# google/neural-light-transport

Hardware: AMD Instinct MI355X
Metric: rendered Mtexels/s at 1024^2 UV (full Model.call forward: U-Net + UV->camera warp); at N > 1: N collective-free replicas of this forward (weak scaling).  The data-parallel TRAIN step with the RCCL gradient all-reduce (BASELINE config 4) is `train_step`: value = Mtexels/s over all ranks, speedup_vs_o (higher is better)
Workload: dtype f32 via 3xbf16 split, 9 exact products, fp32 accumulate (the LDS-tiled encoder convs: fp32 operands as three bf16 terms on v_mfma_f32_16x16x32_bf16, every term product exact in fp32); f32 storage everywhere, every other launch native f32; 1 GPU; BASELINE config 3: dragon_specular relight+view-synth, depth0 16/depth 256, 4 frames/GPU, 1024^2 UV, k=4 obs maps, 512^2 camera warp; frames_per_gpu=4, uv=1024, k=4, cam=512, conv_algo=auto, plan=fused ends, launch=eager, two HIP streams, distinct_batches_rotated=3, launch_tape_replays=0, parallelism=dp1 (frames sharded, no forward collective), world=1, dist_world_size=1, device=cuda:0

## Files before the change

include/nlt_hip.h:

```cpp
#ifndef NLT_HIP_H_
#define NLT_HIP_H_

#ifdef __cplusplus
extern "C" {
#endif

typedef enum {
  NLT_OK = 0,
  NLT_ERR_BAD_ARG = -1,
  NLT_ERR_UNSUPPORTED = -2,
  NLT_ERR_LAUNCH = -3
} nlt_status;

typedef enum {
  NLT_CONV1X1 = 0,
  NLT_CONV_K2S2 = 1,
  NLT_CONV_K2S1 = 2,
  NLT_DECONV_K2S2 = 3,
  NLT_DECONV_K2S1 = 4,
  NLT_CONV_K3S1 = 5,
  NLT_CONV_K3S2 = 6,
  NLT_DECONV_K3S1 = 7,
  NLT_DECONV_K3S2 = 8
} nlt_conv_mode;

typedef enum {
  NLT_ALGO_AUTO = 0,
  NLT_ALGO_DIRECT = 1,
  NLT_ALGO_MFMA = 2
} nlt_conv_algo;

const char* nlt_version(void);
const char* nlt_status_string(int status);

long nlt_packed_weight_floats(int mode, int c0, int c1, int cout);

int nlt_pack_conv_weights(int mode, const float* w_keras, int c0, int c1, int cout,
                          float* w_packed, void* stream);

int nlt_conv_forward(int mode, int algo, int tile_hint,
                     const float* src0, int ld0, int c0,
                     const float* src1, int ld1, int c1,
                     int n, int h, int w,
                     const float* w_keras, const float* w_packed, const float* bias,
                     int cout, float* out, int ldo,
                     int act, float alpha,
                     const float* mask_src, int ldm, int accumulate,
                     void* stream);

int nlt_stem_forward(const float* base, const float* cvis, const float* lvis,
                     const float* nn_rgb, const float* nn_base, const float* obs_weights,
                     int n, int k, int h, int w, int c,
                     const float* wq, const float* bq, const float* wo, const float* bo,
                     float* fm0, float* obs0, void* stream);

int nlt_obs_mean_forward(const float* obs, const float* obs_weights, int n, int k, int hw, int c,
                         float* out, int ldo, void* stream);

int nlt_head_forward(const float* dec, int ldd, int cd, const float* skip, int lds, int cs,
                     const float* w_keras, const float* bias, const float* base,
                     int n, int h, int w, float* pred, void* stream);

int nlt_warp_forward(const float* pred, const float* base, const float* warp,
                     int n, int uvh, int uvw, int hc, int wc,
                     float* pred_cam, float* base_cam, float* fg_cam, int* idx_out, void* stream);

int nlt_warp_forward_store(const float* pred, const unsigned char* diffuse_store, const unsigned short* uv2cam_store,
                           const int* ids, int n, int uvh, int uvw, int hc, int wc,
                           float* pred_cam, float* base_cam, float* fg_cam, int* idx_out, void* stream);

int nlt_resample_forward(const float* data, const float* warp_px, int n, int h, int w, int c, int hc, int wc,
// ... 198 lines not shown
int nlt_front4_forward(const float* base, const float* cvis, const float* lvis, const float* nn_rgb,
                       const float* nn_base, int n, int k, int h, int w, const float* packed,
                       const float* packed_l2, int add_base, float alpha, float* fm1, float* skip3,
                       float* qtmp2, float* otmp2, int waves_per_simd, void* stream);
int nlt_front4_forward_u8(const unsigned char* diffuse_store, const unsigned char* rgb_store,
                          const unsigned char* cvis_store, const unsigned char* lvis_store,
                          const int* ids, const int* nn_ids, int n, int k, int h, int w,
                          const float* packed, const float* packed_l2, int add_base, float alpha,
                          float* fm1, float* skip3, float* qtmp2, float* otmp2, int waves_per_simd, void* stream);

int nlt_front4_forward_train(const float* base, const float* cvis, const float* lvis, const float* nn_rgb,
                             const float* nn_base, int n, int k, int h, int w, const float* packed,
                             const float* packed_l2, int add_base, float alpha, float* fm1, float* skip3,
                             float* qtmp2, float* otmp2, float* obs1, float* qtmp1, float* otmp1, void* stream);

int nlt_dec_block_forward(const float* x, int cx, const float* skip, int cs, int n, int h, int w,
                          const float* w_s2, const float* b_s2, const float* w_s1, const float* b_s1,
                          int c, float alpha, float* out, void* stream);

int nlt_back_forward(const float* x, const float* fm1, const float* skip3, int n, int h2, int w2,
                     const float* w_s2, const float* b_s2, const float* w_s1, const float* b_s1,
                     const float* w_head, float alpha, float* pred, void* stream);

typedef enum { NLT_REPACK_MFMA = 0, NLT_REPACK_TILE = 1, NLT_REPACK_WINO = 2 } nlt_repack_kind;
typedef struct {
  const float* src;
  float* dst;
  long total;
  long first_block;
  int kind, mode;
  int c0, c1, cout;
  int tn;
  int lo, full;
} nlt_repack_desc;
int nlt_repack_weights(const nlt_repack_desc* descs_device, int n_desc, long total_blocks, void* stream);

typedef struct {
  void* fn;
  int n_float, reserved;
  long iargs[32];
  float fargs[4];
} nlt_tape_call;
int nlt_tape_play(const nlt_tape_call* calls, int n, int* failed_index);
int nlt_event_create(int no_system_fence, void** event);
int nlt_event_destroy(void* event);
int nlt_event_record(void* event, void* stream);
int nlt_stream_wait_event(void* stream, void* event);

long nlt_wgrad_narrow_workspace_floats(int mode, int c0, int c1, int n, int h, int w, int cout);
int nlt_conv_backward_weights_narrow(int mode,
                                     const float* src0, int ld0, int c0, const float* src1, int ld1, int c1,
                                     int n, int h, int w, const float* dpre, int ldp, int cout,
                                     float* dw_keras, float* dbias, float* workspace, long workspace_floats,
                                     void* stream);

int nlt_front_forward_train(const float* base, const float* cvis, const float* lvis, const float* nn_rgb,
                            const float* nn_base, int n, int k, int h, int w, const float* packed,
                            int add_base, float alpha, float* fm1, float* obs1, float* skip3,
                            float* qtmp1, float* otmp1, void* stream);
int nlt_back_forward_train(const float* x, const float* fm1, const float* skip3, int n, int h2, int w2,
                           const float* w_s2, const float* b_s2, const float* w_s1, const float* b_s1,
                           const float* w_head, float alpha, float* pred, float* u, float* v, void* stream);

long nlt_front_backward_workspace_floats(int n, int h, int w);
int nlt_front_backward(const float* base, const float* cvis, const float* lvis, const float* nn_rgb,
                       const float* nn_base, int n, int k, int h, int w, const float* dy1q, const float* dy1o,
// ... 109 lines not shown
```

neural-light-transport_amd/_capi.py:

```python
import ctypes
import threading
import os

import torch

_HERE = os.path.dirname(os.path.abspath(__file__))
LIB_PATH = os.environ.get('NLT_HIP_LIB') or os.path.join(_HERE, 'libnlt_hip.so')

CONV1X1, CONV_K2S2, CONV_K2S1, DECONV_K2S2, DECONV_K2S1 = range(5)
CONV_K3S1, CONV_K3S2, DECONV_K3S1, DECONV_K3S2 = range(5, 9)
ALGO_AUTO, ALGO_DIRECT, ALGO_MFMA = range(3)

_c_int, _c_long, _c_float, _vp = ctypes.c_int, ctypes.c_long, ctypes.c_float, ctypes.c_void_p
_c_double = ctypes.c_double
MAP_F64, MAP_F32, MAP_F16 = range(3)

SIGNATURES = {
    'nlt_version': (ctypes.c_char_p, []),
    'nlt_status_string': (ctypes.c_char_p, [_c_int]),
    'nlt_packed_weight_floats': (_c_long, [_c_int] * 4),
    'nlt_pack_conv_weights': (_c_int, [_c_int, _vp, _c_int, _c_int, _c_int, _vp, _vp]),
    'nlt_conv_forward': (_c_int, [_c_int, _c_int, _c_int, _vp, _c_int, _c_int, _vp, _c_int, _c_int,
                                  _c_int, _c_int, _c_int, _vp, _vp, _vp, _c_int, _vp, _c_int,
                                  _c_int, _c_float, _vp, _c_int, _c_int, _vp]),
    'nlt_stem_forward': (_c_int, [_vp] * 6 + [_c_int] * 5 + [_vp] * 4 + [_vp, _vp, _vp]),
    'nlt_obs_mean_forward': (_c_int, [_vp, _vp, _c_int, _c_int, _c_int, _c_int, _vp, _c_int, _vp]),
    'nlt_head_forward': (_c_int, [_vp, _c_int, _c_int, _vp, _c_int, _c_int, _vp, _vp, _vp,
                                  _c_int, _c_int, _c_int, _vp, _vp]),
    'nlt_warp_forward': (_c_int, [_vp, _vp, _vp] + [_c_int] * 5 + [_vp] * 5),
    'nlt_warp_forward_store': (_c_int, [_vp] * 4 + [_c_int] * 5 + [_vp] * 5),
    'nlt_resample_forward': (_c_int, [_vp, _vp] + [_c_int] * 6 + [_vp, _vp]),
    'nlt_resize_bilinear_forward': (_c_int, [_vp] + [_c_int] * 6 + [_vp, _vp]),
    'nlt_mul_forward': (_c_int, [_vp, _vp, _c_long, _vp, _vp]),
    'nlt_conv_backward_weights': (_c_int, [_c_int, _c_int, _vp, _c_int, _c_int, _vp, _c_int, _c_int,
                                           _c_int, _c_int, _c_int, _vp, _c_int, _c_int, _vp, _vp, _vp]),
    'nlt_wgrad_workspace_floats': (_c_long, [_c_int] * 7),
    'nlt_conv_backward_weights_tiled': (_c_int, [_c_int, _vp, _c_int, _c_int, _vp, _c_int, _c_int, _c_int, _c_int, _c_int,
                                                 _vp, _c_int, _c_int, _vp, _vp, _vp, _c_long, _vp]),
    'nlt_repack_weights': (_c_int, [_vp, _c_int, _c_long, _vp]),
    'nlt_tape_play': (_c_int, [_vp, _c_int, _vp]),
    'nlt_event_create': (_c_int, [_c_int, _vp]),
    'nlt_event_destroy': (_c_int, [_vp]),
    'nlt_event_record': (_c_int, [_vp, _vp]),
    'nlt_stream_wait_event': (_c_int, [_vp, _vp]),
    'nlt_wgrad_narrow_workspace_floats': (_c_long, [_c_int] * 7),
    'nlt_conv_backward_weights_narrow': (_c_int, [_c_int, _vp, _c_int, _c_int, _vp, _c_int, _c_int, _c_int, _c_int, _c_int,
                                                 _vp, _c_int, _c_int, _vp, _vp, _vp, _c_long, _vp]),
    'nlt_lrelu_backward': (_c_int, [_vp, _c_int, _vp, _c_int, _c_int, _c_long, _c_float, _vp, _c_int, _vp]),
    'nlt_obs_mean_backward': (_c_int, [_vp, _c_int, _vp, _vp, _vp, _c_int, _c_int, _c_int, _c_int, _c_float, _vp, _vp]),
    'nlt_resize_cv_linear': (_c_int, [_vp, _c_int, _c_int, _c_int, _c_int, _c_int, _c_int, _c_int, _vp, _vp]),
    'nlt_l2_train_loss': (_c_int, [_vp, _vp, _vp, _c_int, _c_long, _c_float, _vp, _vp, _vp, _vp]),
    'nlt_level_split_backward': (_c_int, [_vp, _vp, _c_int, _vp, _vp, _vp, _c_int, _c_int, _c_int, _c_int, _c_float, _c_float, _vp, _vp]),
    'nlt_stem_backward': (_c_int, [_vp] * 6 + [_c_int] * 5 + [_vp] * 6 + [_vp]),
    'nlt_head_backward': (_c_int, [_vp, _c_int, _c_int, _vp, _c_int, _c_int, _vp, _vp, _c_int, _c_int, _c_int,
# ... 408 lines not shown
    if n <= 0:
        raise NLTError("%s%r: unsupported%s" % (name, args, ' (%s)' % what if what else ''))
    return n


_ws_cache = {}
_splitk_ws = _ws_cache


def _workspace(key, device, need, zero=False):
    key = (str(device),) + key if isinstance(key, tuple) else (str(device), key)
    ws = _ws_cache.get(key)
    if ws is None or ws.numel() < need:
        ws = (torch.zeros if zero else torch.empty)(need, device=device, dtype=torch.float32)
        _ws_cache[key] = ws
        _alloc_epoch[0] += 1
    return ws


def _per_stream(family):
    return '%s.%d' % (family, _stream())


def _pack(size_name, size_args, pack_name, pack_args, dtype, device):
    out = torch.empty(_size(size_name, *size_args), device=device, dtype=dtype)
    _call(pack_name, *pack_args, out.data_ptr())
    return out


def packed_weight_floats(mode, c0, c1, cout):
    return lib().nlt_packed_weight_floats(mode, c0, c1, cout)


def pack_conv_weights(mode, w_keras, c0, c1, cout):
    return _pack('nlt_packed_weight_floats', (mode, c0, c1, cout),
                 'nlt_pack_conv_weights', (mode, _ptr(_dense(w_keras, 'w_keras')), c0, c1, cout), torch.float32, w_keras.device)


def conv_forward(mode, src0, c0, ld0, src1, c1, ld1, n, h, w, w_keras, w_packed, bias, cout, out, ldo,
                 act=True, alpha=0.3, algo=ALGO_AUTO, tile_hint=0, mask_src=None, ldm=0, accumulate=False):
    _call('nlt_conv_forward', mode, algo, tile_hint, _ptr(src0), ld0, c0, _ptr(src1), ld1, c1, n, h, w, _ptr(w_keras),
          _ptr(w_packed), _ptr(bias), cout, _ptr(out), ldo, 1 if act else 0, float(alpha), _ptr(mask_src), ldm,
          1 if accumulate else 0)


def stem_forward(base, cvis, lvis, nn_rgb, nn_base, obs_weights, n, k, h, w, c, wq, bq, wo, bo, fm0, obs0):
    for t, nm in ((base, 'base'), (cvis, 'cvis'), (lvis, 'lvis'), (nn_rgb, 'nn_rgb'), (nn_base, 'nn_base')):
        _dense(t, nm)
    _call('nlt_stem_forward', _ptr(base), _ptr(cvis), _ptr(lvis), _ptr(nn_rgb), _ptr(nn_base), _ptr(obs_weights), n, k, h, w, c,
          _ptr(wq), _ptr(bq), _ptr(wo), _ptr(bo), _ptr(fm0), _ptr(obs0))


def obs_mean_forward(obs, obs_weights, n, k, hw, c, out, ldo):
    _call('nlt_obs_mean_forward', _ptr(_dense(obs, 'obs')), _ptr(obs_weights), n, k, hw, c, _ptr(out), ldo)


def head_forward(dec, ldd, cd, skip, lds, cs, w_keras, bias, base, n, h, w, pred):
    _call('nlt_head_forward', _ptr(dec), ldd, cd, _ptr(skip), lds, cs, _ptr(w_keras), _ptr(bias), _ptr(base), n, h, w, _ptr(pred))


def warp_forward(pred, base, warp, n, uvh, uvw, hc, wc, pred_cam, base_cam, fg_cam, idx_out=None):
    _call('nlt_warp_forward', _ptr(pred), _ptr(base), _ptr(_dense(warp, 'warp')), n, uvh, uvw, hc, wc, _ptr(pred_cam),
          _ptr(base_cam), _ptr(fg_cam), _ptr(idx_out))


def warp_forward_store(pred, diffuse_store, uv2cam_store, ids, n, uvh, uvw, hc, wc, pred_cam, base_cam, fg_cam, idx_out=None):
    if tuple(diffuse_store.shape[1:]) != (uvh, uvw, 3) or tuple(uv2cam_store.shape[1:]) != (hc, wc, 2):
# ... 365 lines not shown
    if abs(ksplit) <= 1 and not always:
        return None
    need = _size('nlt_conv_splitk_workspace_floats', mode, n, h, w, cout, ksplit)
    return _workspace((_stream(), getattr(_tls, 'scope', 0)), device, need, zero=True)


def conv_forward_splitk(mode, ksplit, src0, c0, ld0, src1, c1, ld1, n, h, w, w_packed, bias, cout, out, ldo,
                        act=True, alpha=0.3, tile_hint=0, mask_src=None, ldm=0, accumulate=False):
    ws = _splitk_workspace(mode, n, h, w, cout, ksplit, src0.device, always=True)
    _call('nlt_conv_forward_splitk', mode, tile_hint, ksplit, _ptr(ws), _ptr(src0), ld0, c0, _ptr(src1), ld1, c1, n, h, w,
          _ptr(w_packed), _ptr(bias), cout, _ptr(out), ldo, 1 if act else 0, float(alpha), _ptr(mask_src), ldm,
          1 if accumulate else 0)


def conv_forward_map(mode, ksplit, src0, c0, ld0, src1, c1, ld1, n, h, w, w_packed, bias, cout, out, ldo, bias_map,
                     act=True, alpha=0.3, tile_hint=0, w_keras=None):
    ws = _splitk_workspace(mode, n, h, w, cout, ksplit, src0.device)
    _call('nlt_conv_forward_map', mode, tile_hint, ksplit, _ptr(ws), _ptr(src0), ld0, c0, _ptr(src1), ld1, c1, n, h, w,
          _ptr(w_packed), _ptr(bias), cout, _ptr(out), ldo, 1 if act else 0, float(alpha), _ptr(_dense(bias_map, 'bias_map')),
          bias_map.shape[0])


def conv_backward_data(adj_mode, dpre, cpre, ldp, n, h, w, w_packed, zero_bias, cout, out, ldo, mask_src=None, ldm=0,
                       mask_alpha=0.3, accumulate=False, tile_hint=0, ksplit=1, split=None, w_keras=None):
    ws = _splitk_workspace(adj_mode, n, h, w, cout, ksplit, dpre.device)
    sc, sy, sd, sa, sp = split if split is not None else (0, None, None, 0.0, False)
    _call('nlt_conv_backward_data', adj_mode, tile_hint, ksplit, _ptr(ws), _ptr(dpre), ldp, cpre, n, h, w, _ptr(w_packed),
          _ptr(zero_bias), cout, _ptr(out), ldo, _ptr(mask_src), ldm, float(mask_alpha), 1 if accumulate else 0, sc, _ptr(sy),
          _ptr(sd), float(sa), 1 if sp else 0)


REPACK_MFMA, REPACK_TILE, REPACK_WINO = 0, 1, 2
REPACK_FIELDS = [('src', 'u8'), ('dst', 'u8'), ('total', 'i8'), ('first_block', 'i8'), ('kind', 'i4'), ('mode', 'i4'),
                 ('c0', 'i4'), ('c1', 'i4'), ('cout', 'i4'), ('tn', 'i4'), ('lo', 'i4'), ('full', 'i4')]


def repack_table(entries, device):
    import numpy as np
    tab = np.zeros(len(entries), dtype=np.dtype(REPACK_FIELDS))
    blocks = 0
    for i, e in enumerate(entries):
        if e['dst'].numel() % 4 or e['dst'].data_ptr() % 16:
            raise NLTError("repack_table: a packed buffer must be 16-byte aligned and a multiple of 4 floats long")
        tab[i] = (e['src'].data_ptr(), e['dst'].data_ptr(), e['dst'].numel(), blocks, e['kind'], e['mode'], e['c0'], e['c1'],
                  e['cout'], e['tn'], e['lo'], e['full'])
        blocks += (e['dst'].numel() + 255) // 256
    return torch.from_numpy(tab.view(np.uint8)).to(device), len(entries), blocks


def repack_weights(table, n_desc, total_blocks):
    _call('nlt_repack_weights', _tptr(table, torch.uint8, 'repack table'), n_desc, total_blocks)


def conv_tile_supported(mode, cin, cout, tn):
    return lib().nlt_conv_tile_packed_floats(mode, cin, cout, tn) > 0


def pack_conv_tile_weights(mode, w_keras, cin, cout, tn):
    return _pack('nlt_conv_tile_packed_floats', (mode, cin, cout, tn),
                 'nlt_pack_conv_tile_weights', (mode, _ptr(_dense(w_keras, 'w_keras')), cin, cout, tn), torch.float32, w_keras.device)


def conv_tile_forward(mode, src, ld, cin, frames, kobs, h, w, packed, bias, cout, tn, out, ldo, mean_out, ldm,
                      act=True, alpha=0.3):
    _call('nlt_conv_tile_forward', mode, _ptr(src), ld, cin, frames, kobs, h, w, _ptr(packed), _ptr(bias), cout, tn, _ptr(out), ldo,
          _ptr(mean_out), ldm, 1 if act else 0, float(alpha))


def pack_conv_tile_weights_adjoint(adj_mode, w_keras, cpre, cout, tn, full, lo):
    return _pack('nlt_conv_tile_packed_floats', (adj_mode, cpre, cout, tn), 'nlt_pack_conv_tile_weights_adjoint',
                 (adj_mode, _ptr(_dense(w_keras, 'w_keras')), cpre, cout, tn, full, lo), torch.float32, w_keras.device)


def conv_tile_backward_data(adj_mode, dpre, cpre, ldp, n, h, w, packed, cout, tn, out, ldo, mask_src=None, ldm=0, mask_alpha=0.3,
                            accumulate=False, split=None, w_keras=None):
    sc, sy, sd, sa, sp = split if split is not None else (0, None, None, 0.0, False)
    _call('nlt_conv_tile_backward_data', adj_mode, _ptr(dpre), ldp, cpre, n, h, w, _ptr(packed), cout, tn, _ptr(out), ldo,
          _ptr(mask_src), ldm, float(mask_alpha), 1 if accumulate else 0, sc, _ptr(sy), _ptr(sd), float(sa), 1 if sp else 0)
# ... 344 lines not shown
```

neural-light-transport_amd/csrc/conv_mfma.hip:

```cpp
#include "nlt_common.h"
#include "pack_common.h"

namespace {

typedef __attribute__((address_space(1))) unsigned gu32;

__host__ __device__ inline int chunks16(int c) { return (c + 15) >> 4; }

template <int MODE>
__device__ __forceinline__ int keras_widx(int t, int c, int ncol, int cin, int cout) {
  if (MODE == NLT_CONV1X1 || MODE == NLT_CONV_K2S2 || MODE == NLT_CONV_K2S1) return (t * cin + c) * cout + ncol;
  if (MODE == NLT_DECONV_K2S1) return (t * cout + ncol) * cin + c;
  return ncol * cin + c;
}

template <int MODE>
__global__ void pack_weights_kernel(const float* __restrict__ wk, int c0, int c1, int cout, int N,
                                    int ntiles, long total, float* __restrict__ wp) {
  const long idx = (long)blockIdx.x * blockDim.x + threadIdx.x;
  if (idx >= total) return;
  wp[idx] = nlt_mfma_fragment<MODE>(wk, idx, c0, c1, cout, N, ntiles, cout, 0);
}

template <int MODE>
__host__ __device__ inline int live_taps(const ConvP& p) {
  return ((MODE == NLT_CONV_K2S1 || MODE == NLT_DECONV_K2S1) && p.gh == 1 && p.gw == 1) ? 1 : ConvTraits<MODE>::TAPS;
}

__device__ __forceinline__ void split_store(const ConvP& p, int otex, int oc, f32x4 v) {
  const size_t at = (size_t)otex * p.split_c + (oc - p.split_c);
  f32x4* d = reinterpret_cast<f32x4*>(p.split_d + at);
  if (p.split_partial) v += *d;
  const f32x4 mk = *reinterpret_cast<const f32x4*>(p.split_y + at);
#pragma unroll
  for (int j = 0; j < 4; ++j) v[j] *= (mk[j] > 0.f) ? 1.f : p.split_alpha;
  *d = v;
}

template <int MODE, int RT, int CT, int PF, int NW>
__global__ __launch_bounds__(NW ? 64 * NW : 256) void conv_mfma_kernel(ConvP p, int mtiles, int ngroups, int ntiles, int ksplit,
                                                        float* ws) {
  const int lane = threadIdx.x & 63, wv = threadIdx.x >> 6;
  int ng, mt, ks, kg = 0, tile = 0;
  constexpr bool SPLIT = NW > 0;
  if constexpr (SPLIT) {
    const int kgroups = (ksplit + NW - 1) / NW;
    tile = blockIdx.x / kgroups;
    kg = blockIdx.x - tile * kgroups;
    ng = tile % ngroups;
    mt = tile / ngroups;
    ks = kg * NW + wv;
  } else {
    int wave = blockIdx.x * 4 + wv;
    ng = wave % ngroups; wave /= ngroups;
// ... 386 lines not shown
}

}

bool nlt_conv_mfma_supported(int mode, const ConvP& p) {
  (void)mode;
  if ((p.c0 & 3) || (p.c1 & 3) || (p.cout & 3) || (p.ld0 & 3) || (p.ldo & 3)) return false;
  if (p.c1 && (p.ld1 & 3)) return false;
  if (p.mask_src && (p.ldm & 3)) return false;
  if (!nlt_aligned16(p.src0) || !nlt_aligned16(p.out) || !nlt_aligned16(p.bias) || !nlt_aligned16(p.wgt)) return false;
  if (p.c1 && !nlt_aligned16(p.src1)) return false;
  if (p.mask_src && !nlt_aligned16(p.mask_src)) return false;
  return true;
}

int nlt_conv_mfma_launch(int mode, const ConvP& p, int tile_hint, hipStream_t s, int ksplit, float* ws) {
  if (!nlt_conv_mfma_supported(mode, p)) return NLT_ERR_UNSUPPORTED;
  switch (mode) {
    case NLT_CONV1X1: return launch_mode<NLT_CONV1X1>(p, tile_hint, ksplit, ws, s);
    case NLT_CONV_K2S2: return launch_mode<NLT_CONV_K2S2>(p, tile_hint, ksplit, ws, s);
    case NLT_CONV_K2S1: return launch_mode<NLT_CONV_K2S1>(p, tile_hint, ksplit, ws, s);
    case NLT_DECONV_K2S2: return launch_mode<NLT_DECONV_K2S2>(p, tile_hint, ksplit, ws, s);
    case NLT_DECONV_K2S1: return launch_mode<NLT_DECONV_K2S1>(p, tile_hint, ksplit, ws, s);
  }
  return NLT_ERR_BAD_ARG;
}

extern "C" long nlt_packed_weight_floats(int mode, int c0, int c1, int cout) {
  if (mode < NLT_CONV1X1 || mode > NLT_DECONV_K2S1 || c0 <= 0 || c1 < 0 || cout <= 0) return -1;
  const int N = (mode == NLT_DECONV_K2S2) ? 4 * cout : cout;
  return (long)taps_of(mode) * (chunks16(c0) + chunks16(c1)) * ((N + 15) >> 4) * 256;
}

extern "C" int nlt_pack_conv_weights(int mode, const float* w_keras, int c0, int c1, int cout,
                                     float* w_packed, void* stream) {
  if (!w_keras || !w_packed) return NLT_ERR_BAD_ARG;
  const long total = nlt_packed_weight_floats(mode, c0, c1, cout);
  if (total <= 0) return NLT_ERR_BAD_ARG;
  const int N = (mode == NLT_DECONV_K2S2) ? 4 * cout : cout;
  const int ntiles = (N + 15) >> 4;
  hipStream_t s = static_cast<hipStream_t>(stream);
  const unsigned blocks = (unsigned)((total + 255) / 256);
#define NLT_PACK(MODE) hipLaunchKernelGGL(pack_weights_kernel<MODE>, dim3(blocks), dim3(256), 0, s, w_keras, c0, c1, cout, N, ntiles, total, w_packed)
  switch (mode) {
    case NLT_CONV1X1: NLT_PACK(NLT_CONV1X1); break;
    case NLT_CONV_K2S2: NLT_PACK(NLT_CONV_K2S2); break;
    case NLT_CONV_K2S1: NLT_PACK(NLT_CONV_K2S1); break;
    case NLT_DECONV_K2S2: NLT_PACK(NLT_DECONV_K2S2); break;
    case NLT_DECONV_K2S1: NLT_PACK(NLT_DECONV_K2S1); break;
  }
#undef NLT_PACK
  NLT_CHECK_LAUNCH();
  return NLT_OK;
}
```

neural-light-transport_amd/csrc/pack_common.h:

```cpp
#pragma once
#include "nlt_common.h"

__host__ __device__ inline int nlt_chunks16(int c) { return (c + 15) >> 4; }

template <int MODE>
__device__ __forceinline__ long nlt_keras_widx(int t, int c, int ncol, int cin, int cout, int full, int lo) {
  if (MODE == NLT_CONV1X1 || MODE == NLT_CONV_K2S2 || MODE == NLT_CONV_K2S1) return ((long)t * cin + c) * full + lo + ncol;
  if (MODE == NLT_DECONV_K2S1) return ((long)t * full + lo + ncol) * cin + c;
  const int ab = ncol / cout, o = ncol - ab * cout;
  return ((long)ab * full + lo + o) * cin + c;
}

template <int MODE>
__device__ __forceinline__ float nlt_mfma_fragment(const float* __restrict__ wk, long idx, int c0, int c1, int cout, int N,
                                                   int ntiles, int full, int lo) {
  const int s4 = idx & 3;
  const int lane = (idx >> 2) & 63;
  const long tile = idx >> 8;
  const int nt = tile % ntiles;
  const int kc = tile / ntiles;
  const int ch0 = nlt_chunks16(c0), ch1 = nlt_chunks16(c1);
  const int t = kc / (ch0 + ch1);
  const int r = kc % (ch0 + ch1);
  const int s = r >= ch0;
  const int cl = (s ? r - ch0 : r) * 16 + 4 * (lane >> 4) + s4;
  const int cs = s ? c1 : c0;
  const int ncol = nt * 16 + (lane & 15);
  if (cl < cs && ncol < N) return wk[nlt_keras_widx<MODE>(t, (s ? c0 : 0) + cl, ncol, c0 + c1, cout, full, lo)];
  return 0.f;
}

__device__ __forceinline__ float nlt_tile_fragment(const float* __restrict__ wk, long idx, int cin, int cout, int tnt,
                                                   int full, int lo, bool transposed) {
  const int s4 = idx & 3, lane = (idx >> 2) & 63;
  long r = idx >> 8;
  const int ct = r % tnt; r /= tnt;
  const int t = r & 3; r >>= 2;
  const int ncc = cin >> 4;
  const int cc = r % ncc;
  const int g = r / ncc;
  const int c = cc * 16 + 4 * (lane >> 4) + s4;
  const int o = (g * tnt + ct) * 16 + (lane & 15);
  return transposed ? wk[((long)t * full + lo + o) * cin + c] : wk[((long)t * cin + c) * full + lo + o];
}

__device__ __forceinline__ float nlt_tile_fragment_d2(const float* __restrict__ wk, long idx, int cin, int cout, int tnt, int full, int lo) {
  const int s4 = idx & 3, lane = (idx >> 2) & 63;
  long r = idx >> 8;
  const int ct = r % tnt; r /= tnt;
  const int ncc = cin >> 4;
  const int cc = r % ncc;
  const int g = r / ncc;
  const int c = cc * 16 + 4 * (lane >> 4) + s4;
  const int col = (g * tnt + ct) * 16 + (lane & 15);
  const int ab = col / cout, o = col - ab * cout;
  return wk[((long)ab * full + lo + o) * cin + c];
}

__device__ __forceinline__ float nlt_wino_fragment(const float* __restrict__ wk, long idx, int cin, int cout, int tnt,
                                                   int full, int lo, bool transposed) {
  const int e = idx & 3, i = (idx >> 2) & 15, q = (idx >> 6) & 1;
// ... 18 lines not shown
```

neural-light-transport_amd/csrc/repack.hip:

```cpp
#include "pack_common.h"

namespace {

template <int MODE>
__device__ __forceinline__ float frag(const nlt_repack_desc& e, long idx) {
  const int N = MODE == NLT_DECONV_K2S2 ? 4 * e.cout : e.cout;
  return nlt_mfma_fragment<MODE>(e.src, idx, e.c0, e.c1, e.cout, N, (N + 15) >> 4, e.full, e.lo);
}

template <int MODE>
__device__ __forceinline__ f32x4 frag4(const nlt_repack_desc& e, long idx) {
  return (f32x4){frag<MODE>(e, idx), frag<MODE>(e, idx + 1), frag<MODE>(e, idx + 2), frag<MODE>(e, idx + 3)};
}

__global__ __launch_bounds__(64) void repack_all_kernel(const nlt_repack_desc* __restrict__ d, int nd) {
  int lo = 0, hi = nd;
  while (hi - lo > 1) {
    const int mid = (lo + hi) >> 1;
    if (d[mid].first_block <= (long)blockIdx.x) lo = mid; else hi = mid;
  }
  const nlt_repack_desc e = d[lo];
  const long idx = ((long)blockIdx.x - e.first_block) * 256 + threadIdx.x * 4;
  if (idx >= e.total) return;
  f32x4 v;
  if (e.kind == NLT_REPACK_WINO) {
    const bool tr = e.mode == NLT_DECONV_K2S1;
#pragma unroll
    for (int j = 0; j < 4; ++j) v[j] = nlt_wino_fragment(e.src, idx + j, e.c0, e.cout, e.tn >> 4, e.full, e.lo, tr);
  } else if (e.kind == NLT_REPACK_TILE && e.mode == NLT_DECONV_K2S2) {
#pragma unroll
    for (int j = 0; j < 4; ++j) v[j] = nlt_tile_fragment_d2(e.src, idx + j, e.c0, e.cout, e.tn >> 4, e.full, e.lo);
  } else if (e.kind == NLT_REPACK_TILE) {
    const bool tr = e.mode == NLT_DECONV_K2S1 || e.mode == NLT_DECONV_K2S2;
#pragma unroll
    for (int j = 0; j < 4; ++j) v[j] = nlt_tile_fragment(e.src, idx + j, e.c0, e.cout, e.tn >> 4, e.full, e.lo, tr);
  }
  else if (e.mode == NLT_CONV1X1) v = frag4<NLT_CONV1X1>(e, idx);
  else if (e.mode == NLT_CONV_K2S2) v = frag4<NLT_CONV_K2S2>(e, idx);
  else if (e.mode == NLT_CONV_K2S1) v = frag4<NLT_CONV_K2S1>(e, idx);
  else if (e.mode == NLT_DECONV_K2S2) v = frag4<NLT_DECONV_K2S2>(e, idx);
// ... 14 lines not shown
```

neural-light-transport_amd/engine.py:

```python
import os

import torch

from . import _capi as C
from .engine_infer import OverrideMixin


class OpTimer:

    def __init__(self):
        self.pending, self.records = [], {}
        self.flops = {}
        self.moved = {}

    def launch(self, label, nbytes, fn, *args, **kw):
        e0, e1 = torch.cuda.Event(enable_timing=True), torch.cuda.Event(enable_timing=True)
        e0.record()
        fn(*args, **kw)
        e1.record()
        self.pending.append((label, nbytes, e0, e1))

    def collect(self):
        torch.cuda.synchronize()
        for label, nbytes, e0, e1 in self.pending:
# ... 3 lines not shown
        self.pending = []
        return self.records


def _act_kw(act):
    return {'act': act is not None, 'alpha': act.alpha if act is not None else 0.0}


def _gemm(mode, n, h, w, cin, cout):
    ncols = cout * (4 if mode == C.DECONV_K2S2 else 1)
    taps = 4 if mode in (C.CONV_K2S2, C.CONV_K2S1, C.DECONV_K2S1) else 1
    rows = n * h * w // (4 if mode == C.CONV_K2S2 else 1)
    return rows, ncols, 2 * rows * taps * cin * ncols


class RenderPlan(OverrideMixin):
    def __init__(self, net_query, net_obs, use_obs=True):
        self.timer = None
        self.q, self.o, self.use_obs = net_query, net_obs, use_obs
        self.tile_hints = {}
        self.algo_hints = {}
        self.autotune = os.environ.get('NLT_AUTOTUNE', '1') != '0'
        self.fuse_ends = os.environ.get('NLT_FUSED', '1') != '0'
        self._front_blob = None
        self.fuse_override = os.environ.get('NLT_FUSED_OVERRIDE', '1') != '0'
        self._ovr = None
        self.front_l2 = os.environ.get('NLT_FRONT_L2', '1') != '0'
        self.fuse_dec = os.environ.get('NLT_FUSED_DEC', '1') != '0'
        self.front_v4 = os.environ.get('NLT_FRONT4', '1') != '0'
        self.fuse_train = os.environ.get('NLT_FUSED_TRAIN', '1') != '0'
        self.front4_train = os.environ.get('NLT_FRONT4_TRAIN', '1') != '0'
        self.two_streams = os.environ.get('NLT_STREAMS', '2') != '1'
        self._side = None
        self._bside = None
        self.wgrad_tiled = os.environ.get('NLT_WGRAD', 'tiled') != 'atomic'
        self.wgrad_narrow = os.environ.get('NLT_WGRAD_NARROW', '1') != '0'
        self.bwd_streams = int(os.environ.get('NLT_BWD_STREAMS', '1'))
        self.use_tape = os.environ.get('NLT_TAPE', '1') != '0'
        self.fold_split = os.environ.get('NLT_FOLD_SPLIT', '1') != '0'
        self.tile_dgrad = os.environ.get('NLT_TILE_DGRAD', '1') != '0'
        self._tuning = False
        self.tune_backward = os.environ.get('NLT_TUNE_BWD', '1') != '0'
        self.precision = os.environ.get('NLT_PRECISION', 'fp32')
        self._pred_out = None
        self._pred_slot = 'back_infer'
        self.prune_packs = os.environ.get('NLT_PRUNE_PACKS', '1') != '0'
        self.grad_hook = None
        self.grad_mid_level = 0
        self.generation = 0
        self.tape_replays = 0
        self._trial_direct = False
        self._ran_direct = set()
        self._trial_lds = 0
        self._ran_lds = set()
        self.lds_hints = {}
        self.use_wino = os.environ.get('NLT_WINO', '1') != '0'
        self._trial_wino = 0
        self._ran_wino = set()
        self.wino_hints = {}
        self.use_c32 = os.environ.get('NLT_C32', '1') != '0'
        self._trial_c32 = 0
        self._ran_c32 = set()
        self.c32_hints = {}
        self.alias_obs = os.environ.get('NLT_ALIAS_OBS', '1') != '0'
        self._trial_splitk = 0
        self._ran_splitk = set()
        self.splitk_hints = {}
        is_c = net_query.is_contracting
        self.n_down = sum(is_c) - 1
        self.n_up = len(is_c) - sum(is_c) - 1
        assert self.n_down == self.n_up
        self._bufs = {}
# ... 46 lines not shown
            if moved is not None:
                t.moved[label] = moved
        if t is not None and (getattr(t, 'only', None) is None or label in t.only):
            t.launch(label, nbytes, fn, *args, **kw)
        else:
            fn(*args, **kw)

    def _tile_splitk(self, label, rows, ncols, star, trial):
        tile_hint = self.tile_hints.get(label, self.tile_hints.get('*', 0) if star else 0)
        if tile_hint and ((ncols + 15) // 16) % (tile_hint & 15):
            tile_hint = 0
        ks = self.splitk_hints.get(label, 1)
        if trial:
            rt, ct = (tile_hint >> 4, tile_hint & 15) if tile_hint else (1, 1)
            waves = -(-rows // (16 * rt)) * (-(-ncols // 16) // ct)
            npad = -(-ncols // 16) * 16
            ks = self._trial_splitk if (waves < 4096 and rows * npad * abs(self._trial_splitk) <= (1 << 24)) else 1
        return tile_hint, ks

    def _conv(self, label, layer, act, src0, c0, ld0, src1, c1, ld1, n, h, w, out, ldo, algo=C.ALGO_AUTO, bmap=None):
        layer.build(c0 + c1, src0.device)
        assert layer.cin == c0 + c1, (layer.cin, c0, c1)
        small = (c0 + c1) * layer.n_ch_out <= 1024
        if self.algo_hints.get(label) == C.ALGO_DIRECT or (self._trial_direct and small):
            algo = C.ALGO_DIRECT
            self._ran_direct.add(label)
        ok = c0 % 4 == 0 and c1 % 4 == 0 and layer.n_ch_out % 4 == 0 and algo != C.ALGO_DIRECT
        oh, ow = layer.out_hw(h, w)
        nbytes = 4 * (n * h * w * (c0 + c1) + n * oh * ow * layer.n_ch_out)
        rows, ncols, flops = _gemm(layer.mode, n, h, w, c0 + c1, layer.n_ch_out)
        if c1 == 0 and ok and algo == C.ALGO_AUTO and self._wino(label, layer, act, src0, c0, ld0, n, 1, h, w, out, ldo):
            return
        tile_hint, ks = self._tile_splitk(label, rows, ncols, True, self._trial_splitk and ok)
        srcs = (src0, c0, ld0, src1, c1, ld1, n, h, w)
        dst = (layer.bias.detach(), layer.n_ch_out, out, ldo)
        kw = dict(_act_kw(act), flops=flops)
        if bmap is not None:
            if not ok:
                raise C.NLTError("a bias-map conv needs channel counts that are multiples of 4 (%s)" % label)
            if abs(ks) > 1:
                self._ran_splitk.add(label)
            self._launch(label, nbytes, C.conv_forward_map, layer.mode, ks or 1, *srcs, layer.packed(c0, c1), *dst, bmap,
                         tile_hint=tile_hint, w_keras=layer.kernel.detach(), **kw)
        elif abs(ks) > 1 and ok:
            self._ran_splitk.add(label)
            self._launch(label, nbytes, C.conv_forward_splitk, layer.mode, ks, *srcs, layer.packed(c0, c1), *dst,
                         tile_hint=tile_hint, **kw)
        else:
            self._launch(label, nbytes, C.conv_forward, layer.mode, *srcs, layer.kernel.detach(),
                         layer.packed(c0, c1) if ok else None, *dst, algo=algo if ok else C.ALGO_DIRECT,
                         tile_hint=tile_hint if ok else 0, **kw)

    def _mean(self, label, obs, obs_weights, frames, kobs, hw, c, mean_out, ldm):
        self._launch(label.replace('.s1', '.mean'), 4 * frames * hw * c * (kobs + 1), C.obs_mean_forward,
                     obs, obs_weights, frames, kobs, hw, c, mean_out, ldm)

    def _enc_launch(self, fn, packed, extra, ran, unfold, label, layer, act, src, cin, ld, frames, kobs, h, w, out, ldo,
                    mean_out, ldm, **kw):
        oh, ow = layer.out_hw(h, w)
        nf, c = frames * kobs, layer.n_ch_out
        fold_mean = mean_out is not None and not unfold
        nbytes = 4 * (nf * h * w * cin + nf * oh * ow * c)
        if fold_mean:
            nbytes += 4 * frames * oh * ow * c * (kobs + 1)
        ran.add(label)
        self._launch(label, nbytes, fn, layer.mode, src, ld, cin, nf if unfold else frames, 1 if unfold else kobs, h, w, packed,
                     layer.bias.detach(), c, *extra, out, ldo, mean_out if fold_mean else None, ldm, **_act_kw(act), **kw,
                     flops=2 * nf * oh * ow * 4 * cin * c)
        if mean_out is not None and unfold:
            self._mean(label, out, None, frames, kobs, oh * ow, c, mean_out, ldm)

    def _wino(self, label, layer, act, src, cin, ld, frames, kobs, h, w, out, ldo, mean_out=None, ldm=0, obs_weights=None):
        hint = self._trial_wino or self.wino_hints.get(label, 0)
        tn, unfold = hint & 255, bool(hint >> 8)
        if not (tn and self.use_wino and obs_weights is None and layer.mode in (C.CONV_K2S1, C.DECONV_K2S1) and layer.cin == cin
                and cin % 8 == 0 and layer.n_ch_out % tn == 0 and ld % 4 == 0 and ldo % 4 == 0):
            return False
        if layer.mode == C.DECONV_K2S1 and (kobs > 1 or mean_out is not None):
            return False
        if kobs == 1 and mean_out is None:
            if self._trial_wino >> 8:
                return False
            unfold = False
        self._enc_launch(C.conv_wino_forward, layer.packed_wino(tn), (tn,), self._ran_wino, unfold, label, layer, act, src, cin, ld,
                         frames, kobs, h, w, out, ldo, mean_out, ldm)
        return True

    def _conv_bf(self, label, layer, act, src0, c0, ld0, src1, c1, ld1, n, h, w, out, ldo):
# ... 434 lines not shown
            h2_, w2_ = hh // 2, ww // 2

            def obs_path():
                if bf and l >= 3:
                    self._conv_bf('L%d.o.s2' % l, oa, oact_a, b['obs'][l - 1], cl[l - 1], cl[l - 1], None, 0, 0, n * k, hh, ww,
                                  b['otmp'][l], c)
                    self._conv_bf('L%d.o.s1' % l, ob, oact_b, b['otmp'][l], c, c, None, 0, 0, n * k, h2_, w2_, b['obs'][l], c)
                    self._launch('L%d.o.mean' % l, 4 * n * h2_ * w2_ * c * (k + 1), C.obs_mean_bf16, b['obs'][l], n, k, h2_ * w2_, c,
                                 b['fm'][l].view(-1)[c:], 2 * c, moved=2 * n * h2_ * w2_ * c * (k + 1))
                    return
                if alias_obs:
                    if not s2_done:
                        if l > 2:
                            self._conv_enc('L%d.o.s2' % l, oa, oact_a, b['fm'][l - 1].view(-1)[cl[l - 1]:], cl[l - 1], 2 * cl[l - 1],
                                           n, 1, hh, ww, b['otmp'][l], c, algo)
                        else:
                            self._conv_enc('L%d.o.s2' % l, oa, oact_a, b['obs'][1], cl[1], cl[1], n, 1, hh, ww, b['otmp'][l], c, algo)
                    self._conv_enc('L%d.o.s1' % l, ob, oact_b, b['otmp'][l], c, c, n, 1, h2_, w2_, b['fm'][l].view(-1)[c:], 2 * c, algo)
                    return
                if not s2_done:
                    self._conv_enc('L%d.o.s2' % l, oa, oact_a, b['obs'][l - 1], cl[l - 1], cl[l - 1], n, k, hh, ww, b['otmp'][l], c, algo)
                self._conv_enc('L%d.o.s1' % l, ob, oact_b, b['otmp'][l], c, c, n, k, h2_, w2_, b['obs'][l], c, algo,
                               mean_out=b['fm'][l].view(-1)[c:], ldm=2 * c)

            def query_path():
                if bf and l >= 3:
                    self._conv_bf('L%d.q.s2' % l, qa, qact_a, b['fm'][l - 1], cin, cin, None, 0, 0, n, hh, ww, b['qtmp'][l], c)
                    self._conv_bf('L%d.q.s1' % l, qb, qact_b, b['qtmp'][l], c, c, None, 0, 0, n, h2_, w2_, b['fm'][l], 2 * c)
                    return
                if not s2_done:
                    self._conv_enc('L%d.q.s2' % l, qa, qact_a, b['fm'][l - 1], cin, cin, n, 1, hh, ww, b['qtmp'][l], c, algo)
                self._conv_enc('L%d.q.s1' % l, qb, qact_b, b['qtmp'][l], c, c, n, 1, h2_, w2_, b['fm'][l], 2 * c, algo)

            obs_path()
            if concurrent:
                C.record_event(ev[l], main)
                with torch.cuda.stream(side):
                    if l > 2:
                        C.wait_event(side, ev[l - 1])
                    query_path()
            else:
                query_path()
            hh, ww = hh // 2, ww // 2
        if concurrent:
            C.record_event(ev[D + 1], side)
            C.wait_event(main, ev[D + 1])
        x, cx = b['fm'][D], 2 * cl[D]
        for j in range(U - 1):
            (da, dact_a), (db, dact_b) = q.layers[D + 1 + j].convs()
            skip, cs = b['fm'][D - j], 2 * cl[D - j]
            lab = 'L%d.q' % (D + 1 + j)
            nl = da.n_ch_out
            if bf and j <= D - 3:
                self._conv_bf(lab + '.s2', da, dact_a, x, cx, cx, skip, cs, cs, n, hh, ww, b['dtmp'][j], nl)
                hh, ww = hh * 2, ww * 2
                self._conv_bf(lab + '.s1', db, dact_b, b['dtmp'][j], nl, nl, None, 0, 0, n, hh, ww, b['dec'][j], db.n_ch_out)
                x, cx = b['dec'][j], db.n_ch_out
                continue
            if (self.fuse_dec and not train and nl in (8, 16) and db.n_ch_out == nl and cx % 4 == 0 and algo == C.ALGO_AUTO
                    and dact_a is not None and dact_b is not None and dact_a.alpha == dact_b.alpha and not self._trial_direct):
                da.build(cx + cs, dev); db.build(nl, dev)
                nbytes = 4 * n * hh * ww * ((cx + cs) + 4 * nl) + 4 * n * 4 * hh * ww * 2 * nl
                self._launch(lab, nbytes, C.dec_block_forward, x, cx, skip, cs, n, hh, ww, da.kernel.detach(), da.bias.detach(),
                             db.kernel.detach(), db.bias.detach(), nl, dact_a.alpha, b['dec'][j],
                             flops=2 * n * hh * ww * (cx + cs) * 4 * nl + 2 * n * 4 * hh * ww * 4 * nl * nl,
                             moved=4 * n * hh * ww * ((cx + cs) + 4 * nl))
                hh, ww = hh * 2, ww * 2
                x, cx = b['dec'][j], nl
                continue
            x, cx = self._dec_block_plain(b, j, lab, da, dact_a, db, dact_b, (x, cx, cx, skip, cs, cs), n, hh, ww, algo)
            hh, ww = hh * 2, ww * 2
        (da, _), (db, _) = q.layers[D + U].convs()
        head = q.layers[-1]
# ... 295 lines not shown
```

neural-light-transport_amd/networks/elements.py:

```python
import math

import torch

from .. import _capi as C

_seed_counter = [0]


def _glorot_uniform(shape, device, seed):
    kh, kw, a, b = shape
    limit = math.sqrt(6.0 / (kh * kw * a + kh * kw * b))
    g = torch.Generator().manual_seed(seed)
    return ((torch.rand(shape, generator=g) * 2 - 1) * limit).to(device)


class Layer:
    built = True
    trainable = ()

    def build(self, cin, device):
        return cin

    def variables(self):
        return []
# ... 60 lines not shown
    def _version(self):
        return (self.kernel.data_ptr(), self.kernel._version, self._epoch[0])

    def _cached_pack(self, key, make, desc):
        ent = self._packed.get(key)
        ver = self._version()
        reg = self._registry
        if reg is not None:
            reg.touch(self, key)
            if ent is not None and reg.is_inactive(self, key):
                paused = C.tape_pause()
                try:
                    reg.activate(self, key)
                    ent[1].copy_(make())
                finally:
                    C.tape_resume(paused)
                self._packed[key] = (ver, ent[1])
                return ent[1]
        if ent is not None and ent[0] == ver:
            return ent[1]
        if ent is not None and reg is not None and reg.owns(self, key):
            paused = C.tape_pause()
            try:
                reg.refresh()
            finally:
                C.tape_resume(paused)
            return self._packed[key][1]
        buf = make()
        self._packed[key] = (ver, buf)
        if reg is not None:
            reg.add(self, key, buf, desc)
        return buf

    def packed(self, c0, c1):
        return self._cached_pack((c0, c1), lambda: C.pack_conv_weights(self.mode, self.kernel.detach(), c0, c1, self.n_ch_out),
                                 dict(kind=C.REPACK_MFMA, mode=self.mode, c0=c0, c1=c1, cout=self.n_ch_out, tn=0, lo=0,
                                      full=self.n_ch_out))

    def packed_tile(self, tn):
        return self._cached_pack(('tile', tn),
                                 lambda: C.pack_conv_tile_weights(self.mode, self.kernel.detach(), self.cin, self.n_ch_out, tn),
                                 dict(kind=C.REPACK_TILE, mode=self.mode, c0=self.cin, c1=0, cout=self.n_ch_out, tn=tn, lo=0,
                                      full=self.n_ch_out))

    def packed_wino(self, tn):
        return self._cached_pack(('wino', tn),
                                 lambda: C.pack_conv_wino_weights(self.mode, self.kernel.detach(), self.cin, self.n_ch_out, tn),
                                 dict(kind=C.REPACK_WINO, mode=self.mode, c0=self.cin, c1=0, cout=self.n_ch_out, tn=tn, lo=0,
                                      full=self.n_ch_out))

    def packed_adjoint_wino(self, lo, hi, tn):
        adj = self.ADJOINT[self.mode]
        return self._cached_pack(('adjwino', lo, hi, tn),
                                 lambda: C.pack_conv_wino_weights(adj, self.kernel.detach(), self.n_ch_out, hi - lo, tn, self.cin, lo),
                                 dict(kind=C.REPACK_WINO, mode=adj, c0=self.n_ch_out, c1=0, cout=hi - lo, tn=tn, lo=lo, full=self.cin))

    def packed_bf16(self, c0, c1):
        cache = self.__dict__.setdefault('_packed_bf', {})
        ent, ver = cache.get((c0, c1)), self._version()
        if ent is None or ent[0] != ver:
            ent = cache[(c0, c1)] = (ver, C.conv_bf16_pack(self.mode, self.kernel.detach(), c0, c1, self.n_ch_out))
        return ent[1]

    def packed_tile3(self, tn):
        cache = self.__dict__.setdefault('_packed_t3', {})
        ent, ver = cache.get(tn), self._version()
        if ent is None or ent[0] != ver:
            ent = cache[tn] = (ver, C.pack_conv_tile3_weights(self.mode, self.kernel.detach(), self.cin, self.n_ch_out, tn))
        return ent[1]

# ... 348 lines not shown
```

Baseline: 3451 Mtexels/s.

## Fold duplicated concat sources into summed weights and move obs means to side stream

```diff
diff --git a/include/nlt_hip.h b/include/nlt_hip.h
--- a/include/nlt_hip.h
+++ b/include/nlt_hip.h
@@ -37,6 +37,9 @@
 
 int nlt_pack_conv_weights(int mode, const float* w_keras, int c0, int c1, int cout,
                           float* w_packed, void* stream);
+
+int nlt_pack_conv_weights_fold(int mode, const float* w_keras, int c0, int fold, int cout,
+                               float* w_packed, void* stream);
 
 int nlt_conv_forward(int mode, int algo, int tile_hint,
                      const float* src0, int ld0, int c0,
@@ -301,6 +304,8 @@
   int c0, c1, cout;
   int tn;
   int lo, full;
+  int fold;
+  int reserved;
 } nlt_repack_desc;
 int nlt_repack_weights(const nlt_repack_desc* descs_device, int n_desc, long total_blocks, void* stream);
 
diff --git a/neural-light-transport_amd/_capi.py b/neural-light-transport_amd/_capi.py
--- a/neural-light-transport_amd/_capi.py
+++ b/neural-light-transport_amd/_capi.py
@@ -20,6 +20,7 @@
     'nlt_status_string': (ctypes.c_char_p, [_c_int]),
     'nlt_packed_weight_floats': (_c_long, [_c_int] * 4),
     'nlt_pack_conv_weights': (_c_int, [_c_int, _vp, _c_int, _c_int, _c_int, _vp, _vp]),
+    'nlt_pack_conv_weights_fold': (_c_int, [_c_int, _vp, _c_int, _c_int, _c_int, _vp, _vp]),
     'nlt_conv_forward': (_c_int, [_c_int, _c_int, _c_int, _vp, _c_int, _c_int, _vp, _c_int, _c_int,
                                   _c_int, _c_int, _c_int, _vp, _vp, _vp, _c_int, _vp, _c_int,
                                   _c_int, _c_float, _vp, _c_int, _c_int, _vp]),
@@ -494,7 +495,12 @@
     return lib().nlt_packed_weight_floats(mode, c0, c1, cout)
 
 
-def pack_conv_weights(mode, w_keras, c0, c1, cout):
+def pack_conv_weights(mode, w_keras, c0, c1, cout, fold=0):
+    if fold:
+        if c1:
+            raise NLTError("pack_conv_weights: a folded pack has one source (c1 = %d)" % c1)
+        return _pack('nlt_packed_weight_floats', (mode, c0, 0, cout), 'nlt_pack_conv_weights_fold',
+                     (mode, _ptr(_dense(w_keras, 'w_keras')), c0, fold, cout), torch.float32, w_keras.device)
     return _pack('nlt_packed_weight_floats', (mode, c0, c1, cout),
                  'nlt_pack_conv_weights', (mode, _ptr(_dense(w_keras, 'w_keras')), c0, c1, cout), torch.float32, w_keras.device)
 
@@ -926,7 +932,8 @@
 
 REPACK_MFMA, REPACK_TILE, REPACK_WINO = 0, 1, 2
 REPACK_FIELDS = [('src', 'u8'), ('dst', 'u8'), ('total', 'i8'), ('first_block', 'i8'), ('kind', 'i4'), ('mode', 'i4'),
-                 ('c0', 'i4'), ('c1', 'i4'), ('cout', 'i4'), ('tn', 'i4'), ('lo', 'i4'), ('full', 'i4')]
+                 ('c0', 'i4'), ('c1', 'i4'), ('cout', 'i4'), ('tn', 'i4'), ('lo', 'i4'), ('full', 'i4'), ('fold', 'i4'),
+                 ('reserved', 'i4')]
 
 
 def repack_table(entries, device):
@@ -937,7 +944,7 @@
         if e['dst'].numel() % 4 or e['dst'].data_ptr() % 16:
             raise NLTError("repack_table: a packed buffer must be 16-byte aligned and a multiple of 4 floats long")
         tab[i] = (e['src'].data_ptr(), e['dst'].data_ptr(), e['dst'].numel(), blocks, e['kind'], e['mode'], e['c0'], e['c1'],
-                  e['cout'], e['tn'], e['lo'], e['full'])
+                  e['cout'], e['tn'], e['lo'], e['full'], e.get('fold', 0), 0)
         blocks += (e['dst'].numel() + 255) // 256
     return torch.from_numpy(tab.view(np.uint8)).to(device), len(entries), blocks
 
diff --git a/neural-light-transport_amd/csrc/conv_mfma.hip b/neural-light-transport_amd/csrc/conv_mfma.hip
--- a/neural-light-transport_amd/csrc/conv_mfma.hip
+++ b/neural-light-transport_amd/csrc/conv_mfma.hip
@@ -16,10 +16,10 @@
 
 template <int MODE>
 __global__ void pack_weights_kernel(const float* __restrict__ wk, int c0, int c1, int cout, int N,
-                                    int ntiles, long total, float* __restrict__ wp) {
+                                    int ntiles, long total, float* __restrict__ wp, int fold) {
   const long idx = (long)blockIdx.x * blockDim.x + threadIdx.x;
   if (idx >= total) return;
-  wp[idx] = nlt_mfma_fragment<MODE>(wk, idx, c0, c1, cout, N, ntiles, cout, 0);
+  wp[idx] = nlt_mfma_fragment<MODE>(wk, idx, c0, c1, cout, N, ntiles, cout, 0, fold);
 }
 
 template <int MODE>
@@ -472,16 +472,17 @@
   return (long)taps_of(mode) * (chunks16(c0) + chunks16(c1)) * ((N + 15) >> 4) * 256;
 }
 
-extern "C" int nlt_pack_conv_weights(int mode, const float* w_keras, int c0, int c1, int cout,
-                                     float* w_packed, void* stream) {
-  if (!w_keras || !w_packed) return NLT_ERR_BAD_ARG;
+namespace {
+
+int pack_conv_weights(int mode, const float* w_keras, int c0, int c1, int fold, int cout, float* w_packed, void* stream) {
+  if (!w_keras || !w_packed || fold < 0) return NLT_ERR_BAD_ARG;
   const long total = nlt_packed_weight_floats(mode, c0, c1, cout);
   if (total <= 0) return NLT_ERR_BAD_ARG;
   const int N = (mode == NLT_DECONV_K2S2) ? 4 * cout : cout;
   const int ntiles = (N + 15) >> 4;
   hipStream_t s = static_cast<hipStream_t>(stream);
   const unsigned blocks = (unsigned)((total + 255) / 256);
-#define NLT_PACK(MODE) hipLaunchKernelGGL(pack_weights_kernel<MODE>, dim3(blocks), dim3(256), 0, s, w_keras, c0, c1, cout, N, ntiles, total, w_packed)
+#define NLT_PACK(MODE) hipLaunchKernelGGL(pack_weights_kernel<MODE>, dim3(blocks), dim3(256), 0, s, w_keras, c0, c1, cout, N, ntiles, total, w_packed, fold)
   switch (mode) {
     case NLT_CONV1X1: NLT_PACK(NLT_CONV1X1); break;
     case NLT_CONV_K2S2: NLT_PACK(NLT_CONV_K2S2); break;
@@ -493,3 +494,16 @@
   NLT_CHECK_LAUNCH();
   return NLT_OK;
 }
+
+}
+
+extern "C" int nlt_pack_conv_weights(int mode, const float* w_keras, int c0, int c1, int cout,
+                                     float* w_packed, void* stream) {
+  return pack_conv_weights(mode, w_keras, c0, c1, 0, cout, w_packed, stream);
+}
+
+extern "C" int nlt_pack_conv_weights_fold(int mode, const float* w_keras, int c0, int fold, int cout,
+                                          float* w_packed, void* stream) {
+  if (fold <= 0) return NLT_ERR_BAD_ARG;
+  return pack_conv_weights(mode, w_keras, c0, 0, fold, cout, w_packed, stream);
+}
diff --git a/neural-light-transport_amd/csrc/pack_common.h b/neural-light-transport_amd/csrc/pack_common.h
--- a/neural-light-transport_amd/csrc/pack_common.h
+++ b/neural-light-transport_amd/csrc/pack_common.h
@@ -13,7 +13,7 @@
 
 template <int MODE>
 __device__ __forceinline__ float nlt_mfma_fragment(const float* __restrict__ wk, long idx, int c0, int c1, int cout, int N,
-                                                   int ntiles, int full, int lo) {
+                                                   int ntiles, int full, int lo, int fold = 0) {
   const int s4 = idx & 3;
   const int lane = (idx >> 2) & 63;
   const long tile = idx >> 8;
@@ -26,7 +26,10 @@
   const int cl = (s ? r - ch0 : r) * 16 + 4 * (lane >> 4) + s4;
   const int cs = s ? c1 : c0;
   const int ncol = nt * 16 + (lane & 15);
-  if (cl < cs && ncol < N) return wk[nlt_keras_widx<MODE>(t, (s ? c0 : 0) + cl, ncol, c0 + c1, cout, full, lo)];
+  if (cl < cs && ncol < N) {
+    const float v = wk[nlt_keras_widx<MODE>(t, (s ? c0 : 0) + cl, ncol, c0 + c1 + fold, cout, full, lo)];
+    return fold ? v + wk[nlt_keras_widx<MODE>(t, fold + cl, ncol, c0 + c1 + fold, cout, full, lo)] : v;
+  }
   return 0.f;
 }
 
diff --git a/neural-light-transport_amd/csrc/repack.hip b/neural-light-transport_amd/csrc/repack.hip
--- a/neural-light-transport_amd/csrc/repack.hip
+++ b/neural-light-transport_amd/csrc/repack.hip
@@ -5,7 +5,7 @@
 template <int MODE>
 __device__ __forceinline__ float frag(const nlt_repack_desc& e, long idx) {
   const int N = MODE == NLT_DECONV_K2S2 ? 4 * e.cout : e.cout;
-  return nlt_mfma_fragment<MODE>(e.src, idx, e.c0, e.c1, e.cout, N, (N + 15) >> 4, e.full, e.lo);
+  return nlt_mfma_fragment<MODE>(e.src, idx, e.c0, e.c1, e.cout, N, (N + 15) >> 4, e.full, e.lo, e.fold);
 }
 
 template <int MODE>
diff --git a/neural-light-transport_amd/engine.py b/neural-light-transport_amd/engine.py
--- a/neural-light-transport_amd/engine.py
+++ b/neural-light-transport_amd/engine.py
@@ -59,12 +59,15 @@
         self.front4_train = os.environ.get('NLT_FRONT4_TRAIN', '1') != '0'
         self.two_streams = os.environ.get('NLT_STREAMS', '2') != '1'
         self._side = None
+        self.mean_side = os.environ.get('NLT_MEAN_SIDE', '1') != '0'
+        self._held_means = None
         self._bside = None
         self.wgrad_tiled = os.environ.get('NLT_WGRAD', 'tiled') != 'atomic'
         self.wgrad_narrow = os.environ.get('NLT_WGRAD_NARROW', '1') != '0'
         self.bwd_streams = int(os.environ.get('NLT_BWD_STREAMS', '1'))
         self.use_tape = os.environ.get('NLT_TAPE', '1') != '0'
         self.fold_split = os.environ.get('NLT_FOLD_SPLIT', '1') != '0'
+        self.fold_concat = os.environ.get('NLT_FOLD_CONCAT', '1') != '0'
         self.tile_dgrad = os.environ.get('NLT_TILE_DGRAD', '1') != '0'
         self._tuning = False
         self.tune_backward = os.environ.get('NLT_TUNE_BWD', '1') != '0'
@@ -177,7 +180,14 @@
         if c1 == 0 and ok and algo == C.ALGO_AUTO and self._wino(label, layer, act, src0, c0, ld0, n, 1, h, w, out, ldo):
             return
         tile_hint, ks = self._tile_splitk(label, rows, ncols, True, self._trial_splitk and ok)
-        srcs = (src0, c0, ld0, src1, c1, ld1, n, h, w)
+        fold = (self.fold_concat and ok and c1 == c0 and ld1 == ld0 and src1 is not None and src1.data_ptr() == src0.data_ptr()
+                and src1.dtype == src0.dtype)
+        if fold:
+            srcs = (src0, c0, ld0, None, 0, 0, n, h, w)
+            packed, w_keras = layer.packed(c0, c0, fold=True), layer.folded_kernel(c0)
+        else:
+            srcs = (src0, c0, ld0, src1, c1, ld1, n, h, w)
+            packed, w_keras = (layer.packed(c0, c1) if ok else None), layer.kernel.detach()
         dst = (layer.bias.detach(), layer.n_ch_out, out, ldo)
         kw = dict(_act_kw(act), flops=flops)
         if bmap is not None:
@@ -185,20 +195,23 @@
                 raise C.NLTError("a bias-map conv needs channel counts that are multiples of 4 (%s)" % label)
             if abs(ks) > 1:
                 self._ran_splitk.add(label)
-            self._launch(label, nbytes, C.conv_forward_map, layer.mode, ks or 1, *srcs, layer.packed(c0, c1), *dst, bmap,
-                         tile_hint=tile_hint, w_keras=layer.kernel.detach(), **kw)
+            self._launch(label, nbytes, C.conv_forward_map, layer.mode, ks or 1, *srcs, packed, *dst, bmap,
+                         tile_hint=tile_hint, w_keras=w_keras, **kw)
         elif abs(ks) > 1 and ok:
             self._ran_splitk.add(label)
-            self._launch(label, nbytes, C.conv_forward_splitk, layer.mode, ks, *srcs, layer.packed(c0, c1), *dst,
+            self._launch(label, nbytes, C.conv_forward_splitk, layer.mode, ks, *srcs, packed, *dst,
                          tile_hint=tile_hint, **kw)
         else:
-            self._launch(label, nbytes, C.conv_forward, layer.mode, *srcs, layer.kernel.detach(),
-                         layer.packed(c0, c1) if ok else None, *dst, algo=algo if ok else C.ALGO_DIRECT,
-                         tile_hint=tile_hint if ok else 0, **kw)
+            self._launch(label, nbytes, C.conv_forward, layer.mode, *srcs, w_keras, packed, *dst,
+                         algo=C.ALGO_MFMA if fold else (algo if ok else C.ALGO_DIRECT), tile_hint=tile_hint if ok else 0, **kw)
 
     def _mean(self, label, obs, obs_weights, frames, kobs, hw, c, mean_out, ldm):
-        self._launch(label.replace('.s1', '.mean'), 4 * frames * hw * c * (kobs + 1), C.obs_mean_forward,
-                     obs, obs_weights, frames, kobs, hw, c, mean_out, ldm)
+        launch = lambda: self._launch(label.replace('.s1', '.mean'), 4 * frames * hw * c * (kobs + 1), C.obs_mean_forward,
+                                      obs, obs_weights, frames, kobs, hw, c, mean_out, ldm)
+        if self._held_means is not None:
+            self._held_means.append(launch)
+        else:
+            launch()
 
     def _enc_launch(self, fn, packed, extra, ran, unfold, label, layer, act, src, cin, ld, frames, kobs, h, w, out, ldo,
                     mean_out, ldm, **kw):
@@ -699,13 +712,22 @@
                     self._conv_enc('L%d.q.s2' % l, qa, qact_a, b['fm'][l - 1], cin, cin, n, 1, hh, ww, b['qtmp'][l], c, algo)
                 self._conv_enc('L%d.q.s1' % l, qb, qact_b, b['qtmp'][l], c, c, n, 1, h2_, w2_, b['fm'][l], 2 * c, algo)
 
-            obs_path()
+            if concurrent and self.mean_side:
+                self._held_means = []
+            try:
+                obs_path()
+            finally:
+                means, self._held_means = self._held_means, None
             if concurrent:
                 C.record_event(ev[l], main)
                 with torch.cuda.stream(side):
                     if l > 2:
                         C.wait_event(side, ev[l - 1])
                     query_path()
+                    if means:
+                        C.wait_event(side, ev[l])
+                        for launch in means:
+                            launch()
             else:
                 query_path()
             hh, ww = hh // 2, ww // 2
diff --git a/neural-light-transport_amd/networks/elements.py b/neural-light-transport_amd/networks/elements.py
--- a/neural-light-transport_amd/networks/elements.py
+++ b/neural-light-transport_amd/networks/elements.py
@@ -116,10 +116,26 @@
             reg.add(self, key, buf, desc)
         return buf
 
-    def packed(self, c0, c1):
-        return self._cached_pack((c0, c1), lambda: C.pack_conv_weights(self.mode, self.kernel.detach(), c0, c1, self.n_ch_out),
-                                 dict(kind=C.REPACK_MFMA, mode=self.mode, c0=c0, c1=c1, cout=self.n_ch_out, tn=0, lo=0,
-                                      full=self.n_ch_out))
+    def packed(self, c0, c1, fold=False):
+        if not fold:
+            return self._cached_pack((c0, c1), lambda: C.pack_conv_weights(self.mode, self.kernel.detach(), c0, c1, self.n_ch_out),
+                                     dict(kind=C.REPACK_MFMA, mode=self.mode, c0=c0, c1=c1, cout=self.n_ch_out, tn=0, lo=0,
+                                          full=self.n_ch_out))
+        assert c1 == c0 and self.cin == 2 * c0, (self.cin, c0, c1)
+        def make():
+            k = self.folded_kernel(c0)
+            if k is not None:
+                return C.pack_conv_weights(self.mode, k.contiguous(), c0, 0, self.n_ch_out)
+            return C.pack_conv_weights(self.mode, self.kernel.detach(), c0, 0, self.n_ch_out, fold=c0)
+        return self._cached_pack(('fold', c0), make,
+                                 dict(kind=C.REPACK_MFMA, mode=self.mode, c0=c0, c1=0, cout=self.n_ch_out, tn=0, lo=0,
+                                      full=self.n_ch_out, fold=c0))
+
+    def folded_kernel(self, c0):
+        k = self.kernel.detach()
+        if k.is_cuda:
+            return None
+        return (k[..., :c0] + k[..., c0:]) if self.transpose else (k[:, :, :c0, :] + k[:, :, c0:, :])
 
     def packed_tile(self, tn):
         return self._cached_pack(('tile', tn),
```

Result: slower. 3388 Mtexels/s (-1.8%).
